# bjing2016/mdgen

Hardware: AMD Instinct MI355X
Metric: sampled MD frames/sec (higher is better)
Workload: dtype bf16

## Files before the change

### mdgen_amd/csrc/k_flash.hip

```cpp
#include "kernels.h"
#include "panel.h"
#include <type_traits>

namespace mdg {

__device__ __forceinline__ bf16x8 frag16(const unsigned char* p) { return *reinterpret_cast<const bf16x8*>(p); }

__device__ __forceinline__ bf16x8 frag8(const unsigned char* p) {
    const u32x2 v = *reinterpret_cast<const u32x2*>(p);
    const u32x4 w = u32x4{v[0], v[1], 0u, 0u};
    return __builtin_bit_cast(bf16x8, w);
}

struct KTile {
    u32x4 k0;
    u32x4 k1;
};
struct VTile {
    u32x4 v0;
    u32x4 v1;
};
struct QTile {
    bf16x8 q0, q1;
};
// ... 63 lines not shown
        pc.p1[j] = __builtin_amdgcn_perm(__float_as_uint(e[9 + 2 * j]), __float_as_uint(e[8 + 2 * j]), 0x07060302u);
#else
        pc.p0[j] = pack_bf16(e[2 * j], e[2 * j + 1]);
        pc.p1[j] = pack_bf16(e[8 + 2 * j], e[9 + 2 * j]);
#endif
    }
#pragma unroll
    for (int g = 0; g < 4; ++g) {
        __builtin_amdgcn_sched_group_barrier(0x008, 1, 0);
        __builtin_amdgcn_sched_group_barrier(0x402, 6, 0);
    }
    asm volatile("" : "+v"(pc.p0), "+v"(pc.p1) : "v"(k0), "v"(k1), "v"(qn.q0), "v"(qn.q1));
}

constexpr float kDefer = 8.f;

__device__ __forceinline__ void softmax_stats(Half& st, f32x16& s, QTile& q, uint32_t vm, int hh) {
    if (vm != 0xffffffffu) mask_scores(s, vm, hh);
    float t = fmaxf(s[0], s[1]);
#pragma unroll
    for (int r = 2; r < 16; r += 2) t = fmaxf(fmaxf(t, s[r]), s[r + 1]);
    t = half_max(t);
    if ((__builtin_amdgcn_ballot_w64(t > kDefer) | st.unanch) != 0) {
        const bool fin = t > -1e29f;
        const bool un = (st.unanch >> lane_id()) & 1ull;
        const bool mv = (t > kDefer) | (un & fin & (t < -kDefer));
        st.unanch &= ~__builtin_amdgcn_ballot_w64(fin);
        const float r = set_shift(q, mv ? st.m + t : st.m, hh);
        const float e = r - st.m;
        st.m = r;
        const float a = __builtin_amdgcn_exp2f(fminf(-e, 0.f));
#pragma unroll
        for (int i = 0; i < 16; ++i) {
            st.o[i] *= a;
            s[i] -= e;
        }
    }
}

#ifdef MDGEN_DEV_FLASH_STAMPS
__device__ unsigned long long g_flash_stamps[32768 * 16];
extern "C" int mdgen_dev_flash_stamps(void* host, size_t bytes) {
    return (int)hipMemcpyFromSymbol(host, HIP_SYMBOL(g_flash_stamps), bytes);
}
#define FLASH_STAMP(slot, v)                                                                          \
    if (lane == 0 && (long)blockIdx.x * 4 + w < 32768) g_flash_stamps[((long)blockIdx.x * 4 + w) * 16 + (slot)] = (v)
__device__ unsigned long long g_fproj_stamps[8192 * 16];
extern "C" int mdgen_dev_fproj_stamps(void* host, size_t bytes) {
    return (int)hipMemcpyFromSymbol(host, HIP_SYMBOL(g_fproj_stamps), bytes);
}
#define FPROJ_STAMP(slot, v)                                                                          \
    if (lane_id() == 0 && (long)blockIdx.x * 4 + w < 8192) g_fproj_stamps[((long)blockIdx.x * 4 + w) * 16 + (slot)] = (v)
#define FLASH_STAMP_ROW(w, hg) ((w) + 4096 * (hg))
#else
#define FLASH_STAMP(slot, v)
#define FPROJ_STAMP(slot, v)
#define FLASH_STAMP_ROW(w, hg) (w)
#endif

template <int N, class F>
__device__ __forceinline__ void static_for(F&& f) {
    if constexpr (N > 0) {
        static_for<N - 1>(f);
        f(std::integral_constant<int, N - 1>{});
    }
}

struct FlashStoreGlobal {
    __bf16* obuf;
    AxisMap ax;
    int seq, head;
    __device__ __forceinline__ void row(int, int pos, u32x2 a, u32x2 b, u32x2 c) const {
        u32x2* d = reinterpret_cast<u32x2*>(obuf + ax.token(seq, pos) * kC + head * kDH + (lane_id() >> 5) * 12);
        d[0] = a;
        d[1] = b;
        d[2] = c;
    }
    __device__ __forceinline__ void pad(int, int) const {}
};

template <int NQ>
struct FlashPre {
    QTile q[NQ];
    u32x4 kb0;
    u32x2 kb1;
    f32x4 bvl[3];
    KTile k0t;
    uint32_t vmw;
};

__device__ __forceinline__ void* flash_uniform_ptr(const unsigned char* q_) {
    const unsigned long long a = (unsigned long long)q_;
    const unsigned lo = __builtin_amdgcn_readfirstlane((unsigned)a), hi = __builtin_amdgcn_readfirstlane((unsigned)(a >> 32));
    return (void*)(((unsigned long long)hi << 32) | lo);
}

template <int NQ>
__device__ __forceinline__ void flash_prefetch(const FlashParams p, const int seq, const int head, const int qc, FlashPre<NQ>& pre) {
    const int lane = lane_id(), hh = lane >> 5;
    const int len = p.ax.len, nt = p.ax.ntile();
    const long ftile = (long)(seq * kH + head) * nt;
    const unsigned char* qb = p.qf + ftile * kFragQ;
    const int qt0 = NQ * qc;
#pragma unroll
    for (int j = 0; j < NQ; ++j) {
        const int qt = (qt0 + j) * 32 < len ? qt0 + j : qt0;
        pre.q[j].q0 = frag16(qb + (long)qt * kFragQ + lane * 16);
        pre.q[j].q1 = frag8(qb + (long)qt * kFragQ + 1024 + lane * 8);
    }
    const bool bias_alone = (len & 31) == 0 && len >= 32;
// ... 131 lines not shown
    if (bias_alone) {
        const f32x4 b0 = bvl[0], b1 = bvl[1], b2 = bvl[2];
#pragma unroll
        for (int i = 0; i < 4; ++i) {
            vbias[i] = round_bf16(b0[i]);
            vbias[4 + i] = round_bf16(b1[i]);
            vbias[8 + i] = round_bf16(b2[i]);
        }
#pragma unroll
        for (int j = 0; j < NQ; ++j) {
            const u32x4 qa = __builtin_bit_cast(u32x4, q[j].q0);
            const u32x4 qb_ = __builtin_bit_cast(u32x4, q[j].q1);
            float d = 0.f;
#pragma unroll
            for (int i = 0; i < 4; ++i) d += bf16_lo(qa[i]) * bf16_lo(kb0[i]) + bf16_hi(qa[i]) * bf16_hi(kb0[i]);
#pragma unroll
            for (int i = 0; i < 2; ++i) d += bf16_lo(qb_[i]) * bf16_lo(kb1[i]) + bf16_hi(qb_[i]) * bf16_hi(kb1[i]);
            sbias[j] = d + __shfl_xor(d, 32, 64);
        }
    }
    bool robust_needed = p.force_robust != 0;
    {
        const uint32_t vm0 = __builtin_amdgcn_readlane(vmw, 0);
#pragma unroll
        for (int j = 0; j < NQ; ++j) {
            f32x16 s0 = scores(k0t, q[j]);
            if (vm0 != 0xffffffffu) mask_scores(s0, vm0, hh);
            float t0 = fmaxf(s0[0], s0[1]);
#pragma unroll
            for (int r = 2; r < 16; r += 2) t0 = fmaxf(fmaxf(t0, s0[r]), s0[r + 1]);
            t0 = half_max(t0);
            robust_needed |= __builtin_amdgcn_ballot_w64(!(t0 > -1e29f)) != 0;
            h[j].m = set_shift(q[j], t0 + kAnchor, hh);
        }
    }
    FLASH_STAMP(1, __builtin_amdgcn_s_memtime());
    FLASH_STAMP(6, (unsigned long long)robust_needed);
    FLASH_STAMP(8, (unsigned long long)__float_as_uint(h[0].m));
    if (!robust_needed) {
        run(std::false_type{}, nt_fast, (p.rotate && nt_fast > 2 && nt <= 64) ? (qc * nt_fast) / ((len + 32 * NQ - 1) / (32 * NQ)) : 0);
        if (bias_alone) {
#pragma unroll
            for (int j = 0; j < NQ; ++j) {
                const float pb = __builtin_amdgcn_exp2f(sbias[j] - h[j].m);
#pragma unroll
                for (int r = 0; r < 12; ++r) h[j].o[r] += pb * vbias[r];
                if (hh == 0) h[j].o[12] += pb;
            }
        }
        FLASH_STAMP(2, __builtin_amdgcn_s_memtime());
        bool bad = false;
#pragma unroll
        for (int j = 0; j < NQ; ++j) {
            const uint32_t lj = __float_as_uint(h[j].o[12]);
            bad |= (lj & 0x7f800000u) == 0x7f800000u;
            bad |= hh == 0 && (lj & 0x7f800000u) == 0u;
#pragma unroll
            for (int i = 0; i < 16; ++i) bad |= (__float_as_uint(h[j].o[i]) & 0x7f800000u) == 0x7f800000u;
        }
        FLASH_STAMP(9, (unsigned long long)__builtin_amdgcn_ballot_w64(bad));
        robust_needed = __builtin_amdgcn_ballot_w64(bad) != 0;
#ifdef MDGEN_DEV_FLASH_NOFALLBACK
        robust_needed = false;
#endif
    }
    if (robust_needed) {
#pragma unroll
        for (int j = 0; j < NQ; ++j) {
            h[j].m = 0.f;
            h[j].unanch = ~0ull;
            set_shift(q[j], 0.f, hh);
        }
        run(std::true_type{}, nt, 0);
    }
    FLASH_STAMP(3, __builtin_amdgcn_s_memtime());
    FLASH_STAMP(11, (unsigned long long)__float_as_uint(h[0].m));
#ifdef MDGEN_DEV_FLASH_STAMPS
    if (lane == 0 && (long)blockIdx.x * 4 + w < 32768) g_flash_stamps[((long)blockIdx.x * 4 + w) * 16 + 6] |= (unsigned long long)robust_needed << 1;
#endif
#pragma unroll
    for (int j = 0; j < NQ; ++j) {
        const float l = __shfl(h[j].o[12], ql, 64);
        const int pos = (qt0 + j) * 32 + ql;
        if (qvalid[j] && pos < len) {
            const float inv = 1.0f / l;
            const f32x16 o = h[j].o;
            store.row(j, pos, u32x2{pack_bf16(o[0] * inv, o[1] * inv), pack_bf16(o[2] * inv, o[3] * inv)},
                      u32x2{pack_bf16(o[4] * inv, o[5] * inv), pack_bf16(o[6] * inv, o[7] * inv)},
                      u32x2{pack_bf16(o[8] * inv, o[9] * inv), pack_bf16(o[10] * inv, o[11] * inv)});
        } else {
            store.pad(j, pos);
        }
    }
    FLASH_STAMP(5, __builtin_amdgcn_s_memrealtime());
}

template <int NQ>
__global__ __launch_bounds__(256, NQ == 2 ? 3 : 2) void k_flash(const FlashParams p) {
    const int w = __builtin_amdgcn_readfirstlane(wave_id());
    const int nqc = (p.ax.len + 32 * NQ - 1) / (32 * NQ);
    const int xcd = blockIdx.x & 7, rest = blockIdx.x >> 3;
    const int qc = rest % nqc, pair = (rest / nqc) * 8 + xcd;
    const int seq = pair >> 2, hg = pair & 3;
    if (seq >= p.ax.nseq) return;
    const int head = hg * 4 + w;
    FlashPre<NQ> pre;
    flash_prefetch<NQ>(p, seq, head, qc, pre);
    flash_job<NQ>(p, seq, head, qc, w, pre, FlashStoreGlobal{p.obuf, p.ax, seq, head});
}

typedef __attribute__((address_space(3))) unsigned char lds_byte;
struct FlashStorePanel {
    lds_byte* panel;
    int head;
    __device__ __forceinline__ void put(int j, u32x2 a, u32x2 b, u32x2 c) const {
        const int lane = lane_id(), row = 32 * j + (lane & 31), byte = head * 48 + (lane >> 5) * 24;
        typedef __attribute__((address_space(3))) u32x2 lds_u32x2;
        *reinterpret_cast<lds_u32x2*>(panel + panel_off(row, byte, kC * 2)) = a;
        *reinterpret_cast<lds_u32x2*>(panel + panel_off(row, byte + 8, kC * 2)) = b;
        *reinterpret_cast<lds_u32x2*>(panel + panel_off(row, byte + 16, kC * 2)) = c;
    }
    __device__ __forceinline__ void row(int j, int, u32x2 a, u32x2 b, u32x2 c) const { put(j, a, b, c); }
    __device__ __forceinline__ void pad(int j, int) const { put(j, u32x2{0u, 0u}, u32x2{0u, 0u}, u32x2{0u, 0u}); }
};

__global__ __launch_bounds__(256, 2) void k_flash_proj(const FlashProjParams p) {
    constexpr int NQ = 2;
    static_assert(32 * NQ == kPanel, "one workgroup = one 64-row panel");
    __shared__ __attribute__((aligned(16))) unsigned char smem[sizeof(PanelRows) + kPanel * kC * 2];
    PanelRows* pr = reinterpret_cast<PanelRows*>(smem);
    unsigned char* panel = smem + sizeof(PanelRows);
    const int w = __builtin_amdgcn_readfirstlane(wave_id());
    const int nqc = (p.f.ax.len + kPanel - 1) / kPanel;
    const int xcd = blockIdx.x & 7, rest = blockIdx.x >> 3;
    const int qc = rest % nqc, seq = (rest / nqc) * 8 + xcd;
    if (seq >= p.f.ax.nseq) return;
    FPROJ_STAMP(0, __builtin_amdgcn_s_memtime());
    FPROJ_STAMP(8, __builtin_amdgcn_s_memrealtime());
    FPROJ_STAMP(10, (unsigned long long)__builtin_amdgcn_s_getreg((31 << 11) | 4));
    setup_rows_axis(pr, p.f.ax, seq, qc * kPanel, p.mm);
    FlashPre<NQ> cur;
    flash_prefetch<NQ>(p.f, seq, w, qc, cur);
#pragma unroll 1
    for (int hg = 0; hg < 4; ++hg) {
        FlashPre<NQ> nxt;
        flash_prefetch<NQ>(p.f, seq, 4 * (hg < 3 ? hg + 1 : 3) + w, qc, nxt);
        __builtin_amdgcn_sched_barrier(0);
        flash_job<NQ>(p.f, seq, 4 * hg + w, qc, FLASH_STAMP_ROW(w, hg), cur, FlashStorePanel{(lds_byte*)panel, 4 * hg + w});
        cur = nxt;
        FPROJ_STAMP(1 + hg, __builtin_amdgcn_s_memtime());
    }
    __syncthreads();
    FPROJ_STAMP(5, __builtin_amdgcn_s_memtime());
    const int lane = lane_id();
    f32x16 acc[6];
#ifndef MDGEN_DEV_FLASH_NOEARLY
    EpiPre<8> ep;
    epi_rmw_request<8>(0, 0, pr, 96 * w, p.h, ep);
    __builtin_amdgcn_sched_barrier(0);
#endif
    zero_acc<6>(acc);
    wave_gemm<2, 3, 24, false>(panel, kC * 2, 0, 0, p.wo + (size_t)(3 * w) * 24 * 64 + lane, 24 * 64, acc);
    FPROJ_STAMP(6, __builtin_amdgcn_s_memtime());
    __syncthreads();
#ifndef MDGEN_DEV_FLASH_NOEARLY
    epilogue_gate_residual_lds_pre<3>(acc, pr, reinterpret_cast<float*>(panel) + w * (32 * 96), 96 * w, p.bo, p.mm, p.gate_chunk, true,
                                      p.h, ep);
#else
    epilogue_gate_residual_lds<3>(acc, pr, reinterpret_cast<float*>(panel) + w * (32 * 96), 96 * w, p.bo, p.mm, p.gate_chunk, true,
                                  p.h);
#endif
    FPROJ_STAMP(7, __builtin_amdgcn_s_memtime());
    FPROJ_STAMP(9, __builtin_amdgcn_s_memrealtime());
}

__global__ __launch_bounds__(512, 1) void k_flash_proj8(const FlashProjParams p) {
    constexpr int NQ = 4, kRows = 32 * NQ;
    __shared__ __attribute__((aligned(16))) unsigned char smem[2 * sizeof(PanelRows) + kRows * kC * 2];
    PanelRows* pr = reinterpret_cast<PanelRows*>(smem);
    unsigned char* panel = smem + 2 * sizeof(PanelRows);
    const int w8 = __builtin_amdgcn_readfirstlane(wave_id()), g = w8 >> 2, w = w8 & 3;
    const int nqc = (p.f.ax.len + kRows - 1) / kRows;
    const int xcd = blockIdx.x & 7, rest = blockIdx.x >> 3;
    const int qc = rest % nqc, seq = (rest / nqc) * 8 + xcd;
    if (seq >= p.f.ax.nseq) return;
    if (threadIdx.x < kRows) {
        const int hf = threadIdx.x >> 6, i = threadIdx.x & 63;
        const int pos = qc * kRows + hf * kPanel + i;
        long tk = -1, mo = 0;
        if (pos < p.f.ax.len) {
            tk = p.f.ax.token(seq, pos);
            mo = p.mm.row_off(tk);
        }
        pr[hf].tok[i] = (int)tk;
        pr[hf].moff[i] = (int)mo;
        set_uniform(&pr[hf], i, tk, mo);
    }
#pragma unroll 1
    for (int pass = 0; pass < 2; ++pass) {
#ifndef MDGEN_DEV_FLASH_NOPRIO
        if ((w8 >= 4) == (pass == 0)) __builtin_amdgcn_s_setprio(1);
        else __builtin_amdgcn_s_setprio(0);
#endif
        const int head = 8 * pass + w8;
        FlashPre<NQ> pre;
        flash_prefetch<NQ>(p.f, seq, head, qc, pre);
        flash_job<NQ>(p.f, seq, head, qc, w8, pre, FlashStorePanel{(lds_byte*)panel, head});
    }
#ifndef MDGEN_DEV_FLASH_NOPRIO
    __builtin_amdgcn_s_setprio(0);
#endif
    __syncthreads();
    const int lane = lane_id();
    f32x16 acc[6];
#ifndef MDGEN_DEV_FLASH_NOEARLY
    EpiPre<8> ep;
    epi_rmw_request<8>(0, 0, &pr[g], 96 * w, p.h, ep);
    __builtin_amdgcn_sched_barrier(0);
#endif
    zero_acc<6>(acc);
    wave_gemm<2, 3, 24, false>(panel, kC * 2, 2 * g, 0, p.wo + (size_t)(3 * w) * 24 * 64 + lane, 24 * 64, acc);
    __syncthreads();
#ifndef MDGEN_DEV_FLASH_NOEARLY
    epilogue_gate_residual_lds_pre<3>(acc, &pr[g], reinterpret_cast<float*>(panel) + w8 * (32 * 96), 96 * w, p.bo, p.mm, p.gate_chunk, true,
                                      p.h, ep);
#else
    epilogue_gate_residual_lds<3>(acc, &pr[g], reinterpret_cast<float*>(panel) + w8 * (32 * 96), 96 * w, p.bo, p.mm, p.gate_chunk, true,
                                  p.h);
#endif
}

#ifndef MDGEN_FLASH_NQ
#define MDGEN_FLASH_NQ 2
#endif
void launch_flash(const FlashParams& p, hipStream_t s) {
    constexpr int NQ = MDGEN_FLASH_NQ;
    const int nqc = (p.ax.len + 32 * NQ - 1) / (32 * NQ);
    const int npair8 = (p.ax.nseq * 4 + 7) / 8;
    hipLaunchKernelGGL(k_flash<NQ>, dim3(npair8 * nqc * 8), dim3(256), 0, s, p);
}

long flash_proj_jobs(const AxisMap& ax) { return (long)ax.nseq * ((ax.len + kPanel - 1) / kPanel); }

void launch_flash_proj(const FlashProjParams& p, FlashProjForm form, hipStream_t s) {
    const int nseq8 = (p.f.ax.nseq + 7) / 8;
    const int rows = form == FlashProjForm::Q128 ? 2 * kPanel : kPanel;
    const dim3 grid(nseq8 * ((p.f.ax.len + rows - 1) / rows) * 8);
    switch (form) {
    case FlashProjForm::Q128: hipLaunchKernelGGL(k_flash_proj8, grid, dim3(512), 0, s, p); return;
    case FlashProjForm::Q64: hipLaunchKernelGGL(k_flash_proj, grid, dim3(256), 0, s, p); return;
    }
}

}
```

### mdgen_amd/csrc/k_gemm.hip

```cpp
#include "kernels.h"
#include "panel.h"

namespace mdg {

constexpr int kRowB = kC * 2;
constexpr int kPanelBytes = kPanel * kRowB;

constexpr int kRopeLds = kRopeRow + 4;
constexpr int kBiasUnits = 3 * kC / 4;
struct QkvStage {
    float bias[3][kC];
    float rope[kPanel][kRopeLds];
};
struct Attn4Stage {
    float bias[3][kC];
    uint32_t tab[2][kL4Tab];
    float rope[4][kRopeLds];
};
__device__ __forceinline__ const f32x4* stage_bias_src(const QkvParams& p, int u) {
    const float* b = u < kC / 4 ? p.bq : u < 2 * (kC / 4) ? p.bk : p.bv;
    return reinterpret_cast<const f32x4*>(b) + (u % (kC / 4));
}
template <int NT>
struct QkvStager {
// ... 640 lines not shown
            Pf[2 * i + 1] = bf16_hi(u);
        }
    }
    if (PROJ) __syncthreads();
#pragma unroll
    for (int hd = 0; hd < 4; ++hd) {
        const int head = 4 * w + hd;
        const uint32_t* vt = &stage.tab[1][((2 * w + hh) * 4 + hd) * 6];
        float bvv[12];
#pragma unroll
        for (int q = 0; q < 6; ++q) {
            bvv[2 * q] = bf16_lo(vt[q]);
            bvv[2 * q + 1] = bf16_hi(vt[q]);
        }
#pragma unroll
        for (int tt = 0; tt < TT; ++tt) {
            float v[12], o[12];
            head_values<TT>(acc, tt, hd, bb[hd], v);
            dpp_fence(v);
#pragma unroll
            for (int i = 0; i < 12; ++i) o[i] = mul_dpp<1>(v[i], P[tt][hd][1]);
#pragma unroll
            for (int i = 0; i < 12; ++i) o[i] = fmac_dpp<0>(o[i], v[i], P[tt][hd][0]);
#pragma unroll
            for (int i = 0; i < 12; ++i) o[i] = fmac_dpp<2>(o[i], v[i], P[tt][hd][2]);
#pragma unroll
            for (int i = 0; i < 12; ++i) o[i] = fmac_dpp<3>(o[i], v[i], P[tt][hd][3]);
#pragma unroll
            for (int i = 0; i < 12; ++i) o[i] = __builtin_fmaf(P[tt][hd][4], bvv[i], o[i]);
            if (PROJ) {
                const bool ok = tok[tt] >= 0;
#pragma unroll
                for (int i = 0; i < 3; ++i)
                    *reinterpret_cast<u32x2*>(panel + panel_off((t0 + tt) * 32 + tk, head * 48 + hh * 24 + 8 * i, kRowB)) =
                        u32x2{ok ? pack_bf16(o[4 * i], o[4 * i + 1]) : 0u, ok ? pack_bf16(o[4 * i + 2], o[4 * i + 3]) : 0u};
            } else if (tok[tt] >= 0) {
                u32x2* d = reinterpret_cast<u32x2*>(p.obuf + (long)tok[tt] * kC + head * kDH + hh * 12);
                d[0] = u32x2{pack_bf16(o[0], o[1]), pack_bf16(o[2], o[3])};
                d[1] = u32x2{pack_bf16(o[4], o[5]), pack_bf16(o[6], o[7])};
                d[2] = u32x2{pack_bf16(o[8], o[9]), pack_bf16(o[10], o[11])};
            }
        }
        __builtin_amdgcn_sched_barrier(0);
    }
    if (!PROJ) return;
    __syncthreads();
    ATTN4_STAMP(8);
    wave_gemm<TT, 3, 24, false, 4, true>(panel, kRowB, t0, 0, p.wo + (size_t)(3 * w) * 24 * 64 + lane, 24 * 64, acc);
    ATTN4_STAMP(9);
    __syncthreads();
    if constexpr (HALF) {
        float* stage = reinterpret_cast<float*>(panel) + w * (32 * 96);
        epi_stage(acc, stage);
        epi_rmw<8>(0, pr, stage, 96 * w, p.bo, p.mm, p.gate_chunk, true, p.h_rw);
    } else {
        epilogue_gate_residual_lds<3>(acc, pr, reinterpret_cast<float*>(panel) + w * (32 * 96), 96 * w, p.bo, p.mm, p.gate_chunk,
                                      true, p.h_rw);
    }
    ATTN4_STAMP(10);
    ATTN4_STAMP_FLUSH
}

template <int MAXL>
__device__ __forceinline__ void prologue_micro_attn(unsigned char* panel, const PanelRows* pr, const ProjParams& p) {
    const int L = p.ax.len;
    for (int item = threadIdx.x; item < kPanel * kH; item += 256) {
        const int row = item >> 4, head = item & 15;
        const int token = pr->tok[row];
        const int tkc = token < 0 ? 0 : token;
        const int seq = tkc / L;
        const __bf16* sbase = p.qkv_small + (long)seq * L * (3 * kC) + head * kDH;
        const u32x4* qp = reinterpret_cast<const u32x4*>(p.qkv_small + (long)tkc * (3 * kC) + head * kDH);
        u32x4 qv[3], kk[MAXL][3], vv[MAXL][3];
        float mk[MAXL];
#pragma unroll
        for (int i = 0; i < 3; ++i) qv[i] = qp[i];
#pragma unroll
        for (int j = 0; j < MAXL; ++j) {
            const int jc = j < L ? j : L - 1;
            mk[j] = p.mk.at((long)seq * L + jc);
            const u32x4* kp = reinterpret_cast<const u32x4*>(sbase + (long)jc * (3 * kC) + kC);
#pragma unroll
            for (int i = 0; i < 3; ++i) kk[j][i] = kp[i];
        }
        if (MAXL <= 4) {
#pragma unroll
            for (int j = 0; j < MAXL; ++j) {
                const int jc = j < L ? j : L - 1;
                const u32x4* vp = reinterpret_cast<const u32x4*>(sbase + (long)jc * (3 * kC) + 2 * kC);
#pragma unroll
                for (int i = 0; i < 3; ++i) vv[j][i] = vp[i];
            }
        }
        float q[24];
#pragma unroll
        for (int i = 0; i < 3; ++i)
#pragma unroll
            for (int j = 0; j < 4; ++j) {
                q[8 * i + 2 * j] = bf16_lo(qv[i][j]);
                q[8 * i + 2 * j + 1] = bf16_hi(qv[i][j]);
            }
        float s[MAXL + 1];
        float mx = -1e30f;
#pragma unroll
        for (int j = 0; j < MAXL; ++j) {
            float d = 0.f;
#pragma unroll
// ... 311 lines not shown
    __builtin_amdgcn_sched_barrier(0)
#define MLP8_STAMP_FLUSH                                                                      \
    if (lane_id() == 0 && (long)blockIdx.x * 8 + wave_id() < 8192) {                            \
        _Pragma("unroll") for (int k = 0; k < 12; ++k)                                          \
            g_mlp8_stamps[((long)blockIdx.x * 8 + wave_id()) * 16 + k] = m8st[k];               \
    }
#else
#define MLP8_STAMP_DECL
#define MLP8_STAMP(slot)
#define MLP8_STAMP_FLUSH
#endif
template <bool PRE, int S = 1>
__global__ __launch_bounds__(512, 1) void k_mlp8(const MlpParams p) {
    static_assert(kNChunk % (2 * S) == 0, "whole chunks per group");
    __shared__ __attribute__((aligned(16))) unsigned char smem[kPanelBytes + 4 * kPanel * kHRowB];
    __shared__ PanelRows prs;
    __shared__ PanelRows prs2;
    __shared__ int s_last;
    unsigned char* panel = smem;
    PanelRows* pr = &prs;
    const int w8 = __builtin_amdgcn_readfirstlane(wave_id());
    const int g = w8 >> 2, w = w8 & 3;
    const int lane = lane_id(), hh = lane >> 5, tk = lane & 31;
    unsigned char* hb0 = smem + kPanelBytes + (2 * g) * (kPanel * kHRowB);
    unsigned char* hb1 = hb0 + kPanel * kHRowB;
    float* slab = reinterpret_cast<float*>(smem) + w8 * (32 * 96);
    int pn = blockIdx.x, sp = 0;
    if (S > 1) {
        const int xcd = blockIdx.x & 7, rest = blockIdx.x >> 3;
        sp = rest % S;
        pn = (rest / S) * 8 + xcd;
        if ((long)pn * kPanel >= p.nrows) return;
    }
    const int slot = pn * S + sp;
    MLP8_STAMP_DECL;
    MLP8_STAMP(0);
    setup_rows_linear(pr, (long)pn * kPanel, p.nrows, p.mm);
    constexpr bool PRIV = PRE && S > 1;
    if (PRIV) {
        setup_rows_linear(&prs2, (long)pn * kPanel, p.nrows, p.mm);
        if (threadIdx.x < kPanel && prs2.tok[threadIdx.x] >= 0) prs2.tok[threadIdx.x] = slot * kPanel + threadIdx.x;
    }
    __syncthreads();
    if (PRE) {
        if (threadIdx.x < 256) prologue_bf16<kC>(panel, pr, p.o);
        __syncthreads();
        MLP8_STAMP(1);
        f32x16 acc[3];
        zero_acc<3>(acc);
        wave_gemm<1, 3, 24, false>(panel, kRowB, g, 0, p.wo + (size_t)(3 * w) * 24 * 64 + lane, 24 * 64, acc);
        __syncthreads();
        MLP8_STAMP(2);
        epi_stage(acc, slab);
        if (PRIV) epi_rmw<8>(g, pr, slab, 96 * w, p.bo, p.mm, p.gate_chunk_o, true, p.h, &prs2, p.hupd);
        else epi_rmw<8>(g, pr, slab, 96 * w, p.bo, p.mm, p.gate_chunk_o, true, p.h);
        __syncthreads();
    }
    MLP8_STAMP(3);
    const PanelRows* prx = PRIV ? &prs2 : pr;
    const float* hx = PRIV ? p.hupd : p.h;
    if (g == 0) prologue_ln<false, 0, 2>(panel, prx, hx, p.mm, p.shift_chunk, p.scale_chunk, 1e-6f, w, lane);
    else prologue_ln<false, 2, 4>(panel, prx, hx, p.mm, p.shift_chunk, p.scale_chunk, 1e-6f, w, lane);
    __syncthreads();
    MLP8_STAMP(4);
    const bf16x8* w1l = p.w1 + (size_t)w * 24 * 64 + lane;
    const bf16x8* w2l = p.w2 + (size_t)(3 * w) * 96 * 64 + lane;
    const float* b1l = p.b1 + 32 * w + 4 * hh;
    constexpr size_t W1C = (size_t)4 * 24 * 64;
    constexpr int NC = kNChunk / (2 * S);
    const int c0 = NC * (2 * sp + g);
    f32x16 y[6];
    zero_acc<6>(y);
    f32x16 a1[2];
    XPre xp;
    YPre yp;
    {
#pragma unroll
        for (int i = 0; i < kPFX; ++i) xp.w[i] = w1l[(size_t)c0 * W1C + i * 64];
#pragma unroll
        for (int t = 0; t < 2; ++t) xp.a[t] = panel_frag(panel, kRowB, t, 0);
    }
    f32x4 b0;
    zero_acc<2>(a1);
    stage_x<false>(panel, w1l + (size_t)c0 * W1C, xp, a1, b1l + c0 * kHC, b0, nullptr, nullptr, yp);
    {
#pragma unroll
        for (int i = 0; i < kPFX; ++i) xp.w[i] = w1l[(size_t)(c0 + 1) * W1C + i * 64];
#pragma unroll
        for (int t = 0; t < 2; ++t) xp.a[t] = panel_frag(panel, kRowB, t, 0);
        f32x4 b4[4];
#pragma unroll
        for (int a = 0; a < 4; ++a) b4[a] = *reinterpret_cast<const f32x4*>(b1l + c0 * kHC + 8 * a);
        __builtin_amdgcn_sched_barrier(0);
#pragma unroll
        for (int q = 0; q < 8; ++q) gelu_group(a1, b4[q >> 1], hb0, q, w, hh, tk);
    }
    lds_barrier();
    MLP8_STAMP(5);
#pragma unroll 1
    for (int i = 1; i < NC; ++i) {
        const int c = c0 + i;
        unsigned char* hw = (i & 1) ? hb1 : hb0;
        const unsigned char* hr = (i & 1) ? hb0 : hb1;
        zero_acc<2>(a1);
        stage_x<true>(panel, w1l + (size_t)c * W1C, xp, a1, b1l + c * kHC, b0, w2l + (size_t)8 * (c - 1) * 64, hr, yp);
        const int cn = i + 1 < NC ? c + 1 : c;
        stage_y<true>(hr, w2l + (size_t)8 * (c - 1) * 64, yp, y, a1, b0, b1l + c * kHC, hw, w, hh, tk, panel, w1l + (size_t)cn * W1C, xp);
        lds_barrier();
// ... 15 lines not shown
        const float* src = reinterpret_cast<const float*>(smem) + (size_t)((1 - g) * 4 + w) * (3 * 16 * 64);
#pragma unroll
        for (int f = 0; f < 3; ++f)
#pragma unroll
            for (int r = 0; r < 16; ++r) {
                const float lo = g == 0 ? y[f][r] : src[(f * 16 + r) * 64 + lane];
                const float hi = g == 0 ? src[(f * 16 + r) * 64 + lane] : y[3 + f][r];
                z[f][r] = lo + hi;
            }
    }
    MLP8_STAMP(8);
    if (S > 1) {
        float* mine = p.part + ((size_t)slot * 8 + w8) * (3 * 16 * 64) + lane;
#pragma unroll
        for (int f = 0; f < 3; ++f)
#pragma unroll
            for (int r = 0; r < 16; ++r)
                __hip_atomic_store(&mine[(f * 16 + r) * 64], z[f][r], __ATOMIC_RELAXED, __HIP_MEMORY_SCOPE_AGENT);
        asm volatile("s_waitcnt vmcnt(0)" ::: "memory");
        __syncthreads();
        if (threadIdx.x == 0) {
            unsigned* c = p.counters + pn;
            const unsigned old = __hip_atomic_fetch_add(c, 1u, __ATOMIC_RELAXED, __HIP_MEMORY_SCOPE_AGENT);
            s_last = old == (unsigned)(S - 1);
            if (old == (unsigned)(S - 1)) __hip_atomic_store(c, 0u, __ATOMIC_RELAXED, __HIP_MEMORY_SCOPE_AGENT);
        }
        __syncthreads();
        MLP8_STAMP(9);
        if (!s_last) {
            MLP8_STAMP_FLUSH
            return;
        }
        f32x16 zt[3];
#pragma unroll
        for (int f = 0; f < 3; ++f)
#pragma unroll
            for (int r = 0; r < 16; ++r) zt[f][r] = 0.f;
#pragma unroll
        for (int o = 0; o < S; ++o) {
            const float* src = p.part + ((size_t)(pn * S + o) * 8 + w8) * (3 * 16 * 64) + lane;
#pragma unroll
            for (int f = 0; f < 3; ++f)
#pragma unroll
                for (int r = 0; r < 16; ++r)
                    zt[f][r] += __hip_atomic_load(&src[(f * 16 + r) * 64], __ATOMIC_RELAXED, __HIP_MEMORY_SCOPE_AGENT);
        }
#pragma unroll
        for (int f = 0; f < 3; ++f) z[f] = zt[f];
    } else {
        __syncthreads();
    }
    MLP8_STAMP(10);
    epi_stage(z, slab);
    if (PRIV) epi_rmw<8>(g, &prs2, slab, 96 * w, p.b2, p.mm, p.gate_chunk, true, p.hupd, pr, p.h);
    else epi_rmw<8>(g, pr, slab, 96 * w, p.b2, p.mm, p.gate_chunk, true, p.h);
    MLP8_STAMP(11);
    MLP8_STAMP_FLUSH
}

__global__ __launch_bounds__(256, 2) void k_ln_linear(const LnLinearParams p) {
    __shared__ __attribute__((aligned(16))) unsigned char smem[sizeof(PanelRows) + kPanelBytes];
    PanelRows* pr = reinterpret_cast<PanelRows*>(smem);
    unsigned char* panel = smem + sizeof(PanelRows);
    setup_rows_linear(pr, (long)blockIdx.x * kPanel, p.nrows, p.mm);
    __syncthreads();
    prologue_ln<true>(panel, pr, p.h, p.mm, 1, 0, 1e-5f);
    __syncthreads();
    const int w = __builtin_amdgcn_readfirstlane(wave_id()), lane = lane_id(), hh = lane >> 5, n = lane & 31;
    const int ngroups = p.nout / 96;
    for (int g = w; g < ngroups; g += 4) {
        f32x16 acc[6];
        zero_acc<6>(acc);
        wave_gemm<2, 3, 24, false>(panel, kRowB, 0, 0, p.w + (size_t)(3 * g) * 24 * 64 + lane, 24 * 64, acc);
        float b[3];
#pragma unroll
        for (int f = 0; f < 3; ++f) b[f] = p.bias[96 * g + 32 * f + n];
#pragma unroll
        for (int t = 0; t < 2; ++t)
#pragma unroll
            for (int r = 0; r < 16; ++r) {
                const int tk = pr->tok[t * 32 + mfma_row(r, hh)];
                if (tk >= 0) {
                    float* op = p.out + (long)tk * p.nout + 96 * g + n;
#pragma unroll
                    for (int f = 0; f < 3; ++f) op[32 * f] = acc[t * 3 + f][r] + b[f];
                }
            }
        __builtin_amdgcn_sched_barrier(0);
    }
}

__global__ __launch_bounds__(256, 2) void k_final(const FinalParams p) {
    __shared__ __attribute__((aligned(16))) unsigned char smem[sizeof(PanelRows) + kPanelBytes];
    PanelRows* pr = reinterpret_cast<PanelRows*>(smem);
    unsigned char* panel = smem + sizeof(PanelRows);
    setup_rows_linear(pr, (long)blockIdx.x * kPanel, p.nrows, p.mm);
    __syncthreads();
    prologue_ln<false>(panel, pr, p.h, p.mm, p.shift_chunk, p.scale_chunk, 1e-6f);
    __syncthreads();
    const int w = __builtin_amdgcn_readfirstlane(wave_id()), lane = lane_id(), hh = lane >> 5, n = lane & 31;
    if (w < 2) {
        f32x16 acc[1];
        zero_acc<1>(acc);
        wave_gemm<1, 1, 24, false>(panel, kRowB, w, 0, p.w + lane, 24 * 64, acc);
        const bool col_ok = n < p.D;
        const int nc = col_ok ? n : 0;
        const float b = p.bias[nc];
        int tks[16];
// ... 94 lines not shown
```

### mdgen_amd/csrc/panel.h

```cpp
#pragma once
#include "common.h"

namespace mdg {

__device__ __forceinline__ void lds_barrier() { asm volatile("s_waitcnt lgkmcnt(0)\n\ts_barrier" ::: "memory"); }

__device__ __forceinline__ int panel_off(int row, int byte_in_row, int rowb) {
    return row * rowb + (byte_in_row ^ ((row & 15) << 4));
}

__device__ __forceinline__ bf16x8 panel_frag(const unsigned char* panel, const int rowb, int tile, int ks) {
    const int lane = lane_id();
    const int row = tile * 32 + (lane & 31);
    return *reinterpret_cast<const bf16x8*>(panel + panel_off(row, ks * 32 + (lane >> 5) * 16, rowb));
}

template <int TT, int FT, int KSTEPS, bool TRANS, int PF = 4, bool ZC = false>
__device__ __forceinline__ void wave_gemm(const unsigned char* panel, const int rowb, const int tile0, const int ks0,
                                          const bf16x8* __restrict__ wfrag, const int wtile_stride,
                                          f32x16* acc) {
    static_assert(PF < KSTEPS, "prefetch depth");
    bf16x8 wring[PF + 1][FT];
    bf16x8 aring[2][TT];
    const f32x16 zero = {0.f, 0.f, 0.f, 0.f, 0.f, 0.f, 0.f, 0.f, 0.f, 0.f, 0.f, 0.f, 0.f, 0.f, 0.f, 0.f};
// ... 190 lines not shown
#pragma unroll
    for (int it = 0; it < NIT; ++it) {
        const int i = threadIdx.x + 256 * it;
        const int r = i / CPR, c = i % CPR;
        tk[it] = pr->tok[r];
        v[it] = *reinterpret_cast<const u32x4*>(reinterpret_cast<const unsigned char*>(src) +
                                                (long)(tk[it] < 0 ? 0 : tk[it]) * ROWB + c * 16);
    }
#pragma unroll
    for (int it = 0; it < NIT; ++it) {
        const int i = threadIdx.x + 256 * it;
        const int r = i / CPR, c = i % CPR;
        *reinterpret_cast<u32x4*>(panel + panel_off(r, c * 16, ROWB)) = tk[it] >= 0 ? v[it] : u32x4{0u, 0u, 0u, 0u};
    }
}

template <int TT, int FT>
__device__ __forceinline__ void epilogue_gate_residual(const f32x16* acc, const PanelRows* pr, int col0,
                                                       const float* __restrict__ bias, const ModMap mm,
                                                       int gate_chunk, bool gated, float* __restrict__ h) {
    const int lane = lane_id();
    const int hh = lane >> 5, n = lane & 31;
    float b[FT];
#pragma unroll
    for (int f = 0; f < FT; ++f) b[f] = bias[col0 + f * 32 + n];
#pragma unroll
    for (int t = 0; t < TT; ++t) {
#pragma unroll
        for (int r = 0; r < 16; ++r) {
            const int row = t * 32 + mfma_row(r, hh);
            const int tk = pr->tok[row];
            if (tk >= 0) {
                float* hp = h + (long)tk * kC + col0 + n;
                const float* gp = mm.mod + pr->moff[row] + gate_chunk * kC + col0 + n;
#pragma unroll
                for (int f = 0; f < FT; ++f) {
                    const float g = gated ? gp[f * 32] : 1.0f;
                    hp[f * 32] = hp[f * 32] + g * (acc[t * FT + f][r] + b[f]);
                }
            }
        }
    }
}

__device__ __forceinline__ void epi_stage(const f32x16* acc3, float* stage) {
    const int lane = lane_id();
    const int hh = lane >> 5, n = lane & 31;
#pragma unroll
    for (int f = 0; f < 3; ++f)
#pragma unroll
        for (int r = 0; r < 16; ++r) stage[mfma_row(r, hh) * 96 + f * 32 + n] = acc3[f][r];
}

template <int BR>
__device__ __forceinline__ void epi_rmw(const int t, const PanelRows* pr, const float* stage, int col0,
                                        const float* __restrict__ bias, const ModMap mm, int gate_chunk, bool gated,
                                        float* __restrict__ h, const PanelRows* prd = nullptr, float* hd = nullptr) {
    static_assert(16 % BR == 0, "batches of row pairs");
    const int lane = lane_id();
    const int q = lane % 24, r2 = lane / 24;
    const bool active = lane < 48;
    const int slot = active ? lane : 0;
    const f32x4 b4 = *reinterpret_cast<const f32x4*>(bias + col0 + 4 * q);
    const f32x4* stage4 = reinterpret_cast<const f32x4*>(stage);
    const int um = gated ? pr->uniform : -1;
    const bool per_row = gated && um < 0;
    f32x4 gu = f32x4{1.f, 1.f, 1.f, 1.f};
    if (gated && um >= 0) gu = *reinterpret_cast<const f32x4*>(mm.mod + um + gate_chunk * kC + col0 + 4 * q);
#pragma unroll
    for (int b = 0; b < 16 / BR; ++b) {
        f32x4 hv[BR], g[BR];
        int tk[BR], td[BR];
#pragma unroll
        for (int k = 0; k < BR; ++k) {
            const int row = active ? t * 32 + 2 * (BR * b + k) + r2 : 0;
            tk[k] = active ? pr->tok[row] : -1;
            td[k] = prd ? prd->tok[row] : tk[k];
            const long tc = tk[k] < 0 ? 0 : tk[k];
            hv[k] = *reinterpret_cast<const f32x4*>(h + tc * kC + col0 + 4 * q);
            g[k] = gu;
            if (per_row) g[k] = *reinterpret_cast<const f32x4*>(mm.mod + pr->moff[row] + gate_chunk * kC + col0 + 4 * q);
        }
#pragma unroll
        for (int k = 0; k < BR; ++k) {
            const f32x4 v = stage4[(BR * b + k) * 48 + slot];
            f32x4 o = hv[k];
            o[0] += g[k][0] * (v[0] + b4[0]);
            o[1] += g[k][1] * (v[1] + b4[1]);
            o[2] += g[k][2] * (v[2] + b4[2]);
            o[3] += g[k][3] * (v[3] + b4[3]);
            if (tk[k] >= 0) *reinterpret_cast<f32x4*>((hd ? hd : h) + (long)td[k] * kC + col0 + 4 * q) = o;
        }
    }
}

template <int BR>
struct EpiPre {
    f32x4 hv[BR];
    int tk[BR];
};
template <int BR>
__device__ __forceinline__ void epi_rmw_request(const int t, const int b, const PanelRows* pr, int col0, const float* __restrict__ h,
                                                EpiPre<BR>& e) {
    const int lane = lane_id();
    const int q = lane % 24, r2 = lane / 24;
    const bool active = lane < 48;
#pragma unroll
    for (int k = 0; k < BR; ++k) {
        const int row = active ? t * 32 + 2 * (BR * b + k) + r2 : 0;
        e.tk[k] = active ? pr->tok[row] : -1;
        const long tc = e.tk[k] < 0 ? 0 : e.tk[k];
        e.hv[k] = *reinterpret_cast<const f32x4*>(h + tc * kC + col0 + 4 * q);
    }
}
template <int BR>
__device__ __forceinline__ void epi_rmw_finish(const int b, const float* stage, int col0, const f32x4 b4, const f32x4 gu,
                                               float* __restrict__ h, const EpiPre<BR>& e) {
    const int lane = lane_id();
    const int q = lane % 24;
    const int slot = lane < 48 ? lane : 0;
    const f32x4* stage4 = reinterpret_cast<const f32x4*>(stage);
#pragma unroll
    for (int k = 0; k < BR; ++k) {
        const f32x4 v = stage4[(BR * b + k) * 48 + slot];
        f32x4 o = e.hv[k];
        o[0] += gu[0] * (v[0] + b4[0]);
        o[1] += gu[1] * (v[1] + b4[1]);
        o[2] += gu[2] * (v[2] + b4[2]);
        o[3] += gu[3] * (v[3] + b4[3]);
        if (e.tk[k] >= 0) *reinterpret_cast<f32x4*>(h + (long)e.tk[k] * kC + col0 + 4 * q) = o;
    }
}
template <int FT>
__device__ __forceinline__ void epilogue_gate_residual_lds_pre(const f32x16* acc, const PanelRows* pr, float* stage, int col0,
                                                               const float* __restrict__ bias, const ModMap mm, int gate_chunk,
                                                               bool gated, float* __restrict__ h, EpiPre<8>& e0) {
    static_assert(FT == 3, "slab is [32][96]");
    const int um = gated ? pr->uniform : -1;
    if (um < 0) {
#pragma unroll
        for (int t = 0; t < 2; ++t) {
            epi_stage(acc + t * FT, stage);
            epi_rmw<8>(t, pr, stage, col0, bias, mm, gate_chunk, gated, h);
        }
        return;
    }
    const int q = lane_id() % 24;
    const f32x4 b4 = *reinterpret_cast<const f32x4*>(bias + col0 + 4 * q);
    const f32x4 gu = *reinterpret_cast<const f32x4*>(mm.mod + um + gate_chunk * kC + col0 + 4 * q);
    EpiPre<8> e1;
    epi_stage(acc, stage);
    epi_rmw_request<8>(0, 1, pr, col0, h, e1);
    __builtin_amdgcn_sched_barrier(0);
    epi_rmw_finish<8>(0, stage, col0, b4, gu, h, e0);
    __builtin_amdgcn_sched_barrier(0);
    epi_rmw_request<8>(1, 0, pr, col0, h, e0);
    __builtin_amdgcn_sched_barrier(0);
    epi_rmw_finish<8>(1, stage, col0, b4, gu, h, e1);
    __builtin_amdgcn_sched_barrier(0);
    epi_stage(acc + FT, stage);
    epi_rmw_request<8>(1, 1, pr, col0, h, e1);
    __builtin_amdgcn_sched_barrier(0);
    epi_rmw_finish<8>(0, stage, col0, b4, gu, h, e0);
    __builtin_amdgcn_sched_barrier(0);
    epi_rmw_finish<8>(1, stage, col0, b4, gu, h, e1);
}

template <int FT>
__device__ __forceinline__ void epilogue_gate_residual_lds(const f32x16* acc, const PanelRows* pr, float* stage, int col0,
                                                           const float* __restrict__ bias, const ModMap mm,
                                                           int gate_chunk, bool gated, float* __restrict__ h) {
    static_assert(FT == 3, "slab is [32][96]");
#pragma unroll
    for (int t = 0; t < 2; ++t) {
        epi_stage(acc + t * FT, stage);
        epi_rmw<8>(t, pr, stage, col0, bias, mm, gate_chunk, gated, h);
    }
}

}
```

Baseline: 125,800.

## Use all 64 lanes in gated residual epilogue via rotated column mapping

```diff
diff --git a/mdgen_amd/csrc/k_flash.hip b/mdgen_amd/csrc/k_flash.hip
--- a/mdgen_amd/csrc/k_flash.hip
+++ b/mdgen_amd/csrc/k_flash.hip
@@ -139,10 +139,26 @@
 #define FPROJ_STAMP(slot, v)                                                                          \
     if (lane_id() == 0 && (long)blockIdx.x * 4 + w < 8192) g_fproj_stamps[((long)blockIdx.x * 4 + w) * 16 + (slot)] = (v)
 #define FLASH_STAMP_ROW(w, hg) ((w) + 4096 * (hg))
+#define FLASH_STAMP_ROW8(w8, pass) ((int)blockIdx.x * 12 + 8 * (pass) + (w8))
+#define FPROJ8_STAMPS unsigned long long st8[7], rt8[2]
+#define FPROJ8_MARK(i) st8[i] = __builtin_amdgcn_s_memtime()
+#define FPROJ8_REAL(i) rt8[i] = __builtin_amdgcn_s_memrealtime()
+#define FPROJ8_FLUSH(w8)                                                              \
+    if (lane_id() == 0 && (long)blockIdx.x * 8 + (w8) < 8192) {                       \
+        unsigned long long* d = g_fproj_stamps + ((long)blockIdx.x * 8 + (w8)) * 16;  \
+        for (int i = 0; i < 7; ++i) d[i] = st8[i];                                    \
+        d[8] = rt8[0];                                                                \
+        d[9] = rt8[1];                                                                \
+    }
 #else
 #define FLASH_STAMP(slot, v)
 #define FPROJ_STAMP(slot, v)
 #define FLASH_STAMP_ROW(w, hg) (w)
+#define FLASH_STAMP_ROW8(w8, pass) (w8)
+#define FPROJ8_STAMPS
+#define FPROJ8_MARK(i)
+#define FPROJ8_REAL(i)
+#define FPROJ8_FLUSH(w8)
 #endif
 
 template <int N, class F>
@@ -380,11 +396,11 @@
         bool bad = false;
 #pragma unroll
         for (int j = 0; j < NQ; ++j) {
-            const uint32_t lj = __float_as_uint(h[j].o[12]);
-            bad |= (lj & 0x7f800000u) == 0x7f800000u;
-            bad |= hh == 0 && (lj & 0x7f800000u) == 0u;
-#pragma unroll
-            for (int i = 0; i < 16; ++i) bad |= (__float_as_uint(h[j].o[i]) & 0x7f800000u) == 0x7f800000u;
+            bad |= hh == 0 && (__float_as_uint(h[j].o[12]) & 0x7f800000u) == 0u;
+            uint32_t big = 0u;
+#pragma unroll
+            for (int i = 0; i < 16; ++i) big = max(big, __float_as_uint(h[j].o[i]) & 0x7fffffffu);
+            bad |= big >= 0x7f800000u;
         }
         FLASH_STAMP(9, (unsigned long long)__builtin_amdgcn_ballot_w64(bad));
         robust_needed = __builtin_amdgcn_ballot_w64(bad) != 0;
@@ -421,6 +437,7 @@
         }
     }
     FLASH_STAMP(5, __builtin_amdgcn_s_memrealtime());
+    FLASH_STAMP(7, __builtin_amdgcn_s_memtime());
 }
 
 template <int NQ>
@@ -483,8 +500,8 @@
     const int lane = lane_id();
     f32x16 acc[6];
 #ifndef MDGEN_DEV_FLASH_NOEARLY
-    EpiPre<8> ep;
-    epi_rmw_request<8>(0, 0, pr, 96 * w, p.h, ep);
+    EpiPre<6> ep;
+    epi_rmw_request<6>(0, 0, pr, 96 * w, p.h, ep);
     __builtin_amdgcn_sched_barrier(0);
 #endif
     zero_acc<6>(acc);
@@ -512,6 +529,9 @@
     const int xcd = blockIdx.x & 7, rest = blockIdx.x >> 3;
     const int qc = rest % nqc, seq = (rest / nqc) * 8 + xcd;
     if (seq >= p.f.ax.nseq) return;
+    FPROJ8_STAMPS;
+    FPROJ8_MARK(0);
+    FPROJ8_REAL(0);
     if (threadIdx.x < kRows) {
         const int hf = threadIdx.x >> 6, i = threadIdx.x & 63;
         const int pos = qc * kRows + hf * kPanel + i;
@@ -533,22 +553,27 @@
         const int head = 8 * pass + w8;
         FlashPre<NQ> pre;
         flash_prefetch<NQ>(p.f, seq, head, qc, pre);
-        flash_job<NQ>(p.f, seq, head, qc, w8, pre, FlashStorePanel{(lds_byte*)panel, head});
+        flash_job<NQ>(p.f, seq, head, qc, FLASH_STAMP_ROW8(w8, pass), pre, FlashStorePanel{(lds_byte*)panel, head});
+        if (pass == 0) FPROJ8_MARK(1);
+        else FPROJ8_MARK(2);
     }
 #ifndef MDGEN_DEV_FLASH_NOPRIO
     __builtin_amdgcn_s_setprio(0);
 #endif
     __syncthreads();
+    FPROJ8_MARK(3);
     const int lane = lane_id();
     f32x16 acc[6];
 #ifndef MDGEN_DEV_FLASH_NOEARLY
-    EpiPre<8> ep;
-    epi_rmw_request<8>(0, 0, &pr[g], 96 * w, p.h, ep);
+    EpiPre<6> ep;
+    epi_rmw_request<6>(0, 0, &pr[g], 96 * w, p.h, ep);
     __builtin_amdgcn_sched_barrier(0);
 #endif
     zero_acc<6>(acc);
     wave_gemm<2, 3, 24, false>(panel, kC * 2, 2 * g, 0, p.wo + (size_t)(3 * w) * 24 * 64 + lane, 24 * 64, acc);
+    FPROJ8_MARK(4);
     __syncthreads();
+    FPROJ8_MARK(5);
 #ifndef MDGEN_DEV_FLASH_NOEARLY
     epilogue_gate_residual_lds_pre<3>(acc, &pr[g], reinterpret_cast<float*>(panel) + w8 * (32 * 96), 96 * w, p.bo, p.mm, p.gate_chunk, true,
                                       p.h, ep);
@@ -556,6 +581,9 @@
     epilogue_gate_residual_lds<3>(acc, &pr[g], reinterpret_cast<float*>(panel) + w8 * (32 * 96), 96 * w, p.bo, p.mm, p.gate_chunk, true,
                                   p.h);
 #endif
+    FPROJ8_MARK(6);
+    FPROJ8_REAL(1);
+    FPROJ8_FLUSH(w8);
 }
 
 #ifndef MDGEN_FLASH_NQ
diff --git a/mdgen_amd/csrc/k_gemm.hip b/mdgen_amd/csrc/k_gemm.hip
--- a/mdgen_amd/csrc/k_gemm.hip
+++ b/mdgen_amd/csrc/k_gemm.hip
@@ -716,7 +716,7 @@
     if constexpr (HALF) {
         float* stage = reinterpret_cast<float*>(panel) + w * (32 * 96);
         epi_stage(acc, stage);
-        epi_rmw<8>(0, pr, stage, 96 * w, p.bo, p.mm, p.gate_chunk, true, p.h_rw);
+        epi_rmw<6>(0, pr, stage, 96 * w, p.bo, p.mm, p.gate_chunk, true, p.h_rw);
     } else {
         epilogue_gate_residual_lds<3>(acc, pr, reinterpret_cast<float*>(panel) + w * (32 * 96), 96 * w, p.bo, p.mm, p.gate_chunk,
                                       true, p.h_rw);
@@ -1134,8 +1134,8 @@
         __syncthreads();
         MLP8_STAMP(2);
         epi_stage(acc, slab);
-        if (PRIV) epi_rmw<8>(g, pr, slab, 96 * w, p.bo, p.mm, p.gate_chunk_o, true, p.h, &prs2, p.hupd);
-        else epi_rmw<8>(g, pr, slab, 96 * w, p.bo, p.mm, p.gate_chunk_o, true, p.h);
+        if (PRIV) epi_rmw<6>(g, pr, slab, 96 * w, p.bo, p.mm, p.gate_chunk_o, true, p.h, &prs2, p.hupd);
+        else epi_rmw<6>(g, pr, slab, 96 * w, p.bo, p.mm, p.gate_chunk_o, true, p.h);
         __syncthreads();
     }
     MLP8_STAMP(3);
@@ -1257,8 +1257,8 @@
     }
     MLP8_STAMP(10);
     epi_stage(z, slab);
-    if (PRIV) epi_rmw<8>(g, &prs2, slab, 96 * w, p.b2, p.mm, p.gate_chunk, true, p.hupd, pr, p.h);
-    else epi_rmw<8>(g, pr, slab, 96 * w, p.b2, p.mm, p.gate_chunk, true, p.h);
+    if (PRIV) epi_rmw<6>(g, &prs2, slab, 96 * w, p.b2, p.mm, p.gate_chunk, true, p.hupd, pr, p.h);
+    else epi_rmw<6>(g, pr, slab, 96 * w, p.b2, p.mm, p.gate_chunk, true, p.h);
     MLP8_STAMP(11);
     MLP8_STAMP_FLUSH
 }
diff --git a/mdgen_amd/csrc/panel.h b/mdgen_amd/csrc/panel.h
--- a/mdgen_amd/csrc/panel.h
+++ b/mdgen_amd/csrc/panel.h
@@ -266,118 +266,131 @@
         for (int r = 0; r < 16; ++r) stage[mfma_row(r, hh) * 96 + f * 32 + n] = acc3[f][r];
 }
 
-template <int BR>
+struct EpiLane {
+    int q[3];
+    __device__ __forceinline__ EpiLane() {
+        const int q0 = lane_id() % 24;
+        q[0] = q0;
+        q[1] = q0 < 8 ? q0 + 16 : q0 - 8;
+        q[2] = q0 < 16 ? q0 + 8 : q0 - 16;
+    }
+    __device__ __forceinline__ int row(int k) const { return (64 * k + lane_id()) / 24; }
+};
+template <int NB>
 __device__ __forceinline__ void epi_rmw(const int t, const PanelRows* pr, const float* stage, int col0,
                                         const float* __restrict__ bias, const ModMap mm, int gate_chunk, bool gated,
                                         float* __restrict__ h, const PanelRows* prd = nullptr, float* hd = nullptr) {
-    static_assert(16 % BR == 0, "batches of row pairs");
+    static_assert(12 % NB == 0 && NB % 3 == 0, "batches of whole three-instruction groups");
     const int lane = lane_id();
-    const int q = lane % 24, r2 = lane / 24;
-    const bool active = lane < 48;
-    const int slot = active ? lane : 0;
-    const f32x4 b4 = *reinterpret_cast<const f32x4*>(bias + col0 + 4 * q);
+    const EpiLane el;
     const f32x4* stage4 = reinterpret_cast<const f32x4*>(stage);
     const int um = gated ? pr->uniform : -1;
     const bool per_row = gated && um < 0;
-    f32x4 gu = f32x4{1.f, 1.f, 1.f, 1.f};
-    if (gated && um >= 0) gu = *reinterpret_cast<const f32x4*>(mm.mod + um + gate_chunk * kC + col0 + 4 * q);
-#pragma unroll
-    for (int b = 0; b < 16 / BR; ++b) {
-        f32x4 hv[BR], g[BR];
-        int tk[BR], td[BR];
-#pragma unroll
-        for (int k = 0; k < BR; ++k) {
-            const int row = active ? t * 32 + 2 * (BR * b + k) + r2 : 0;
-            tk[k] = active ? pr->tok[row] : -1;
+    f32x4 b4[3], gu[3];
+#pragma unroll
+    for (int m = 0; m < 3; ++m) {
+        b4[m] = *reinterpret_cast<const f32x4*>(bias + col0 + 4 * el.q[m]);
+        gu[m] = f32x4{1.f, 1.f, 1.f, 1.f};
+        if (gated && um >= 0) gu[m] = *reinterpret_cast<const f32x4*>(mm.mod + um + gate_chunk * kC + col0 + 4 * el.q[m]);
+    }
+#pragma unroll
+    for (int b = 0; b < 12 / NB; ++b) {
+        f32x4 hv[NB], g[NB];
+        int tk[NB], td[NB];
+#pragma unroll
+        for (int k = 0; k < NB; ++k) {
+            const int q = el.q[k % 3], row = t * 32 + el.row(NB * b + k);
+            tk[k] = pr->tok[row];
             td[k] = prd ? prd->tok[row] : tk[k];
             const long tc = tk[k] < 0 ? 0 : tk[k];
             hv[k] = *reinterpret_cast<const f32x4*>(h + tc * kC + col0 + 4 * q);
-            g[k] = gu;
+            g[k] = gu[k % 3];
             if (per_row) g[k] = *reinterpret_cast<const f32x4*>(mm.mod + pr->moff[row] + gate_chunk * kC + col0 + 4 * q);
         }
 #pragma unroll
-        for (int k = 0; k < BR; ++k) {
-            const f32x4 v = stage4[(BR * b + k) * 48 + slot];
+        for (int k = 0; k < NB; ++k) {
+            const f32x4 v = stage4[(NB * b + k) * 64 + lane], bk = b4[k % 3];
             f32x4 o = hv[k];
-            o[0] += g[k][0] * (v[0] + b4[0]);
-            o[1] += g[k][1] * (v[1] + b4[1]);
-            o[2] += g[k][2] * (v[2] + b4[2]);
-            o[3] += g[k][3] * (v[3] + b4[3]);
-            if (tk[k] >= 0) *reinterpret_cast<f32x4*>((hd ? hd : h) + (long)td[k] * kC + col0 + 4 * q) = o;
-        }
-    }
-}
-
-template <int BR>
+            o[0] += g[k][0] * (v[0] + bk[0]);
+            o[1] += g[k][1] * (v[1] + bk[1]);
+            o[2] += g[k][2] * (v[2] + bk[2]);
+            o[3] += g[k][3] * (v[3] + bk[3]);
+            if (tk[k] >= 0) *reinterpret_cast<f32x4*>((hd ? hd : h) + (long)td[k] * kC + col0 + 4 * el.q[k % 3]) = o;
+        }
+    }
+}
+
+template <int NB>
 struct EpiPre {
-    f32x4 hv[BR];
-    int tk[BR];
+    f32x4 hv[NB];
+    int tk[NB];
 };
-template <int BR>
+template <int NB>
 __device__ __forceinline__ void epi_rmw_request(const int t, const int b, const PanelRows* pr, int col0, const float* __restrict__ h,
-                                                EpiPre<BR>& e) {
+                                                EpiPre<NB>& e) {
+    static_assert(12 % NB == 0 && NB % 3 == 0, "batches of whole three-instruction groups");
+    const EpiLane el;
+#pragma unroll
+    for (int k = 0; k < NB; ++k) {
+        e.tk[k] = pr->tok[t * 32 + el.row(NB * b + k)];
+        const long tc = e.tk[k] < 0 ? 0 : e.tk[k];
+        e.hv[k] = *reinterpret_cast<const f32x4*>(h + tc * kC + col0 + 4 * el.q[k % 3]);
+    }
+}
+template <int NB>
+__device__ __forceinline__ void epi_rmw_finish(const int b, const float* stage, int col0, const f32x4* b4, const f32x4* gu,
+                                               float* __restrict__ h, const EpiPre<NB>& e) {
     const int lane = lane_id();
-    const int q = lane % 24, r2 = lane / 24;
-    const bool active = lane < 48;
-#pragma unroll
-    for (int k = 0; k < BR; ++k) {
-        const int row = active ? t * 32 + 2 * (BR * b + k) + r2 : 0;
-        e.tk[k] = active ? pr->tok[row] : -1;
-        const long tc = e.tk[k] < 0 ? 0 : e.tk[k];
-        e.hv[k] = *reinterpret_cast<const f32x4*>(h + tc * kC + col0 + 4 * q);
-    }
-}
-template <int BR>
-__device__ __forceinline__ void epi_rmw_finish(const int b, const float* stage, int col0, const f32x4 b4, const f32x4 gu,
-                                               float* __restrict__ h, const EpiPre<BR>& e) {
-    const int lane = lane_id();
-    const int q = lane % 24;
-    const int slot = lane < 48 ? lane : 0;
+    const EpiLane el;
     const f32x4* stage4 = reinterpret_cast<const f32x4*>(stage);
 #pragma unroll
-    for (int k = 0; k < BR; ++k) {
-        const f32x4 v = stage4[(BR * b + k) * 48 + slot];
+    for (int k = 0; k < NB; ++k) {
+        const f32x4 v = stage4[(NB * b + k) * 64 + lane], bk = b4[k % 3], gk = gu[k % 3];
         f32x4 o = e.hv[k];
-        o[0] += gu[0] * (v[0] + b4[0]);
-        o[1] += gu[1] * (v[1] + b4[1]);
-        o[2] += gu[2] * (v[2] + b4[2]);
-        o[3] += gu[3] * (v[3] + b4[3]);
-        if (e.tk[k] >= 0) *reinterpret_cast<f32x4*>(h + (long)e.tk[k] * kC + col0 + 4 * q) = o;
+        o[0] += gk[0] * (v[0] + bk[0]);
+        o[1] += gk[1] * (v[1] + bk[1]);
+        o[2] += gk[2] * (v[2] + bk[2]);
+        o[3] += gk[3] * (v[3] + bk[3]);
+        if (e.tk[k] >= 0) *reinterpret_cast<f32x4*>(h + (long)e.tk[k] * kC + col0 + 4 * el.q[k % 3]) = o;
     }
 }
 template <int FT>
 __device__ __forceinline__ void epilogue_gate_residual_lds_pre(const f32x16* acc, const PanelRows* pr, float* stage, int col0,
                                                                const float* __restrict__ bias, const ModMap mm, int gate_chunk,
-                                                               bool gated, float* __restrict__ h, EpiPre<8>& e0) {
+                                                               bool gated, float* __restrict__ h, EpiPre<6>& e0) {
     static_assert(FT == 3, "slab is [32][96]");
     const int um = gated ? pr->uniform : -1;
     if (um < 0) {
 #pragma unroll
         for (int t = 0; t < 2; ++t) {
             epi_stage(acc + t * FT, stage);
-            epi_rmw<8>(t, pr, stage, col0, bias, mm, gate_chunk, gated, h);
+            epi_rmw<6>(t, pr, stage, col0, bias, mm, gate_chunk, gated, h);
         }
         return;
     }
-    const int q = lane_id() % 24;
-    const f32x4 b4 = *reinterpret_cast<const f32x4*>(bias + col0 + 4 * q);
-    const f32x4 gu = *reinterpret_cast<const f32x4*>(mm.mod + um + gate_chunk * kC + col0 + 4 * q);
-    EpiPre<8> e1;
+    const EpiLane el;
+    f32x4 b4[3], gu[3];
+#pragma unroll
+    for (int m = 0; m < 3; ++m) {
+        b4[m] = *reinterpret_cast<const f32x4*>(bias + col0 + 4 * el.q[m]);
+        gu[m] = *reinterpret_cast<const f32x4*>(mm.mod + um + gate_chunk * kC + col0 + 4 * el.q[m]);
+    }
+    EpiPre<6> e1;
     epi_stage(acc, stage);
-    epi_rmw_request<8>(0, 1, pr, col0, h, e1);
-    __builtin_amdgcn_sched_barrier(0);
-    epi_rmw_finish<8>(0, stage, col0, b4, gu, h, e0);
-    __builtin_amdgcn_sched_barrier(0);
-    epi_rmw_request<8>(1, 0, pr, col0, h, e0);
-    __builtin_amdgcn_sched_barrier(0);
-    epi_rmw_finish<8>(1, stage, col0, b4, gu, h, e1);
+    epi_rmw_request<6>(0, 1, pr, col0, h, e1);
+    __builtin_amdgcn_sched_barrier(0);
+    epi_rmw_finish<6>(0, stage, col0, b4, gu, h, e0);
+    __builtin_amdgcn_sched_barrier(0);
+    epi_rmw_request<6>(1, 0, pr, col0, h, e0);
+    __builtin_amdgcn_sched_barrier(0);
+    epi_rmw_finish<6>(1, stage, col0, b4, gu, h, e1);
     __builtin_amdgcn_sched_barrier(0);
     epi_stage(acc + FT, stage);
-    epi_rmw_request<8>(1, 1, pr, col0, h, e1);
-    __builtin_amdgcn_sched_barrier(0);
-    epi_rmw_finish<8>(0, stage, col0, b4, gu, h, e0);
-    __builtin_amdgcn_sched_barrier(0);
-    epi_rmw_finish<8>(1, stage, col0, b4, gu, h, e1);
+    epi_rmw_request<6>(1, 1, pr, col0, h, e1);
+    __builtin_amdgcn_sched_barrier(0);
+    epi_rmw_finish<6>(0, stage, col0, b4, gu, h, e0);
+    __builtin_amdgcn_sched_barrier(0);
+    epi_rmw_finish<6>(1, stage, col0, b4, gu, h, e1);
 }
 
 template <int FT>
@@ -388,8 +401,8 @@
 #pragma unroll
     for (int t = 0; t < 2; ++t) {
         epi_stage(acc + t * FT, stage);
-        epi_rmw<8>(t, pr, stage, col0, bias, mm, gate_chunk, gated, h);
-    }
-}
-
-}
+        epi_rmw<6>(t, pr, stage, col0, bias, mm, gate_chunk, gated, h);
+    }
+}
+
+}
```

New measurement: 126,500, median of 6. No clear change (+0.6%).
